# magenta/ddsp

Hardware: NVIDIA H100
Metric: audio samples/sec (Harmonic+FilteredNoise decoder) (higher is better)
Workload: dtype f32

## Files before the change

ddsp_b200/csrc/capi.cu:

```cuda
#include <stdarg.h>
#include <string.h>

#include <algorithm>

#include "common.cuh"
#include "controls.cuh"
#include "harmonic.cuh"
#include "harmonic_common.cuh"
#include "harmonic_v4.cuh"
#include "noise.cuh"
#include "noise_fused.cuh"
#include "noise_ring.cuh"
#include "host_pipeline.cuh"
#include "backward.cuh"
#include "harmonic_bwd2.cuh"
#include "controls_bwd.cuh"
#include "oscbank.cuh"
#include "sinusoidal.cuh"
#include "longconv.cuh"
#include "spectral.cuh"

namespace ddsp {

static thread_local char g_err[512] = "";
// ... 790 lines not shown
  const size_t z = (size_t)B * g.n_in * lc::M, h = (size_t)ir_batch * g.P * lc::M,
               w = (size_t)B * g.w_len;
  return sizeof(float2) * (z + h + w) + 256;
}

int ddsp_b200_fft_convolve_lti(const float* audio, const float* impulse_response,
                               float* out, int B, int N, int S, int ir_batch,
                               int start, int out_len, int accumulate, int flags,
                               void* workspace, size_t workspace_bytes, void* stream) {
  DDSP_REQUIRE(audio && impulse_response && out, DDSP_B200_E_INVALID,
               "fft_convolve_lti: null pointer");
  DDSP_REQUIRE(B >= 0 && N >= 1 && S >= 1, DDSP_B200_E_INVALID,
               "fft_convolve_lti: bad shape B=%d N=%d S=%d", B, N, S);
  DDSP_REQUIRE(ir_batch == B || ir_batch == 1, DDSP_B200_E_INVALID,
               "Batch size of audio (%d) and impulse response (%d) must be the same.",
               B, ir_batch);
  DDSP_REQUIRE(start >= 0 && out_len >= 0 &&
                   (long long)start + out_len <= (long long)N + S - 1,
               DDSP_B200_E_INVALID,
               "fft_convolve_lti: crop [%d, %d) leaves the convolution of length %lld",
               start, start + out_len, (long long)N + S - 1);
  if (B == 0 || out_len == 0) return 0;
  DDSP_REQUIRE(B <= 65535, DDSP_B200_E_INVALID,
               "fft_convolve_lti: B=%d exceeds the 65535 grid limit", B);
  const size_t need = ddsp_b200_fft_convolve_lti_workspace(B, N, S, ir_batch);
  DDSP_REQUIRE(workspace != nullptr && workspace_bytes >= need, DDSP_B200_E_WORKSPACE,
               "fft_convolve_lti: workspace of %zu B needed, %zu given", need,
               workspace_bytes);
  const lc::Geom g = lc::geom(N, S);
  float2* Z = reinterpret_cast<float2*>(((uintptr_t)workspace + 255) & ~(uintptr_t)255);
  float2* H = Z + (size_t)B * g.n_in * lc::M;
  float2* W = H + (size_t)ir_batch * g.P * lc::M;
  cudaStream_t st = (cudaStream_t)stream;
  DDSP_REQUIRE((flags & ~3) == 0, DDSP_B200_E_INVALID,
               "fft_convolve_lti: bad flags %d", flags);
  lc::lc_fft_blocks<<<dim3(g.P, ir_batch), lc::THREADS, 0, st>>>(
      impulse_response, H, S, 0, g.P, 1, (flags & DDSP_B200_LTI_REVERSE_IR) ? 1 : 0);
  DDSP_CHECK_LAUNCH("fft_convolve_lti(ir spectra)");
  lc::lc_fft_blocks<<<dim3(g.n_in, B), lc::THREADS, 0, st>>>(
      audio, Z, N, g.n2, g.n_in, 0, (flags & DDSP_B200_LTI_REVERSE_AUDIO) ? 1 : 0);
  DDSP_CHECK_LAUNCH("fft_convolve_lti(audio spectra)");
  const int lo_pos = std::max(0, start - g.n2);
  const int hi_pos = std::min(g.w_len, start + out_len);
  const int j_first = lo_pos / lc::L;
  const int j_last = std::min(g.n_out - 1, (hi_pos - 1) / lc::L);
  const int n_blocks = j_last - j_first + 1;
  {
    int rc = set_smem(lc::lc_mac_ifft, lc::kMacSmem, "fft_convolve_lti");
    if (rc) return rc;
  }
  lc::lc_mac_ifft<<<dim3((n_blocks + lc::JT - 1) / lc::JT, B), lc::THREADS, lc::kMacSmem,
                    st>>>(
      Z, H, W, g.n_in, g.P, g.n_out, ir_batch == 1 ? 0 : g.P * lc::M, j_first, n_blocks);
  DDSP_CHECK_LAUNCH("fft_convolve_lti(multiply-accumulate + inverse)");
  const int cgrid = std::min((out_len + 255) / 256, 8 * num_sms());
  lc::lc_combine<<<dim3(cgrid, B), 256, 0, st>>>(W, out, g.n2, g.w_len, start, out_len,
                                               N + S - 1, accumulate, j_first * lc::L,
                                               (j_last + 1) * lc::L);
  DDSP_CHECK_LAUNCH("fft_convolve_lti(combine)");
  return 0;
}

int ddsp_b200_angular_cumsum(const float* angular_frequency, float* phase, int B,
                             int N, int C, int chunk_size, int mode,
                             void* workspace, size_t workspace_bytes, void* stream) {
  DDSP_REQUIRE(angular_frequency && phase, DDSP_B200_E_INVALID,
               "angular_cumsum: null pointer");
  DDSP_REQUIRE(B >= 0 && N >= 1 && C >= 1, DDSP_B200_E_INVALID,
               "angular_cumsum: bad shape B=%d N=%d C=%d", B, N, C);
  DDSP_REQUIRE(mode >= 0 && mode <= 2, DDSP_B200_E_INVALID,
               "angular_cumsum: bad mode %d", mode);
  DDSP_REQUIRE(mode != 2 || chunk_size >= 1, DDSP_B200_E_INVALID,
               "angular_cumsum: chunk_size must be positive");
  if (B == 0) return 0;
  cudaStream_t st = (cudaStream_t)stream;
  if (mode != 0) {
    const int64_t BC = (int64_t)B * C;
    tf_sequential_cumsum<<<(int)((BC + 127) / 128), 128, 0, st>>>(
        angular_frequency, nullptr, phase, B, N, C, mode, chunk_size, 0, 1.0f);
    DDSP_CHECK_LAUNCH("angular_cumsum(tf_sequential)");
    return 0;
  }
  DDSP_REQUIRE(B <= 65535, DDSP_B200_E_INVALID,
               "angular_cumsum: B=%d exceeds the 65535 grid limit", B);
  const size_t need = ddsp_b200_oscillator_bank_workspace(B, N, C);
  DDSP_REQUIRE(workspace != nullptr && workspace_bytes >= need, DDSP_B200_E_WORKSPACE,
               "angular_cumsum: workspace of %zu B needed, %zu given", need,
               workspace_bytes);
  unsigned long long* sums = reinterpret_cast<unsigned long long*>(
      ((uintptr_t)workspace + 255) & ~(uintptr_t)255);
  const int n_chunks = (N + kObChunk - 1) / kObChunk;
  const double inv_two_pi = 0.15915494309189535;
  dim3 grid(n_chunks, B);
  oscbank_chunk_sums<<<grid, kObThreads, 0, st>>>(angular_frequency, sums, N, C,
                                                 n_chunks, inv_two_pi);
  DDSP_CHECK_LAUNCH("angular_cumsum(chunk sums)");
  const int64_t BK = (int64_t)B * C;
  oscbank_scan_chunks<<<(int)((BK + kObThreads - 1) / kObThreads), kObThreads, 0, st>>>(
      sums, C, n_chunks, BK);
  DDSP_CHECK_LAUNCH("angular_cumsum(scan)");
  oscbank_phase_out<<<grid, kObThreads, 0, st>>>(angular_frequency, sums, phase, N, C,
                                                n_chunks, inv_two_pi);
  DDSP_CHECK_LAUNCH("angular_cumsum(apply)");
  return 0;
}

int ddsp_b200_oscillator_bank_tf_sequential(const float* frequency_envelopes,
                                            const float* amplitude_envelopes,
                                            float* out, int B, int N, int K,
                                            float sample_rate, int use_angular_cumsum,
                                            int chunk_size, void* stream) {
  DDSP_REQUIRE(frequency_envelopes && amplitude_envelopes && out, DDSP_B200_E_INVALID,
               "oscillator_bank_tf_sequential: null pointer");
  DDSP_REQUIRE(B >= 0 && N >= 1 && K >= 1 && chunk_size >= 1 && sample_rate > 0.f,
               DDSP_B200_E_INVALID, "oscillator_bank_tf_sequential: bad arguments");
  if (B == 0) return 0;
  const int64_t BK = (int64_t)B * K;
  tf_sequential_cumsum<<<(int)((BK + 127) / 128), 128, 0, (cudaStream_t)stream>>>(
      frequency_envelopes, amplitude_envelopes, out, B, N, K,
      use_angular_cumsum ? 2 : 1, chunk_size, 1, sample_rate);
  DDSP_CHECK_LAUNCH("oscillator_bank_tf_sequential");
  return 0;
}

static int sinus_tile_frames(int F, int K) {
  int FT = std::min(16, F);
  while (FT > 1 && sf_smem(FT, K).total > kMaxDynSmem) FT = (FT + 1) / 2;
  return FT;
}

size_t ddsp_b200_sinusoidal_workspace(int B, int F, int K) {
  if (B <= 0 || F <= 0 || K <= 0) return 0;
  const int FT = sinus_tile_frames(F, K);
  const size_t n_tiles = ((size_t)F + FT - 1) / FT;
  return sizeof(unsigned long long) * (size_t)B * n_tiles * K + 256;
}

int ddsp_b200_sinusoidal_forward(const float* frequencies, const float* amplitudes,
                                 float* audio, int B, int F, int K, int N,
                                 float sample_rate, int amp_method, int accumulate,
                                 void* workspace, size_t workspace_bytes,
                                 void* stream) {
  DDSP_REQUIRE(frequencies && amplitudes && audio, DDSP_B200_E_INVALID,
               "sinusoidal_forward: null pointer");
  DDSP_REQUIRE(B >= 0 && F >= 1 && K >= 1 && N >= 1, DDSP_B200_E_INVALID,
               "sinusoidal_forward: bad shape B=%d F=%d K=%d N=%d", B, F, K, N);
  DDSP_REQUIRE(amp_method == DDSP_B200_AMP_WINDOW || amp_method == DDSP_B200_AMP_LINEAR,
               DDSP_B200_E_INVALID, "sinusoidal_forward: bad amp_method %d", amp_method);
  DDSP_REQUIRE(N % F == 0, DDSP_B200_E_INVALID,
               "sinusoidal_forward: n_samples (%d) must be divisible by the number "
               "of frames (%d)", N, F);
  DDSP_REQUIRE(amp_method != DDSP_B200_AMP_WINDOW || F < N, DDSP_B200_E_INVALID,
               "sinusoidal_forward: window upsampling cannot downsample (frames %d "
               ">= timesteps %d)", F, N);
  DDSP_REQUIRE(sample_rate > 0.f, DDSP_B200_E_INVALID,
               "sinusoidal_forward: sample_rate must be positive");
  if (B == 0) return 0;
  DDSP_REQUIRE(B <= 65535, DDSP_B200_E_INVALID,
               "sinusoidal_forward: B=%d exceeds the 65535 grid limit", B);
  const int FT = sinus_tile_frames(F, K);
  const SfSmem L = sf_smem(FT, K);
  DDSP_REQUIRE(L.total <= kMaxDynSmem, DDSP_B200_E_UNSUPPORTED,
               "sinusoidal_forward: K=%d needs more shared memory than one CTA has", K);
  const size_t need = ddsp_b200_sinusoidal_workspace(B, F, K);
  DDSP_REQUIRE(workspace != nullptr && workspace_bytes >= need, DDSP_B200_E_WORKSPACE,
               "sinusoidal_forward: workspace of %zu B needed, %zu given", need,
               workspace_bytes);
  unsigned long long* sums = reinterpret_cast<unsigned long long*>(
      ((uintptr_t)workspace + 255) & ~(uintptr_t)255);
  const int n_tiles = (F + FT - 1) / FT;
  const int hop = N / F;
  const double inv_sr = 1.0 / (double)sample_rate;
  cudaStream_t st = (cudaStream_t)stream;
  dim3 grid(n_tiles, B);
  sinus_tile_sums<<<grid, kSfThreads, 0, st>>>(frequencies, sums, F, K, hop, FT, n_tiles,
                                              inv_sr);
  DDSP_CHECK_LAUNCH("sinusoidal_forward(tile sums)");
  const int64_t BK = (int64_t)B * K;
  oscbank_scan_chunks<<<(int)((BK + kObThreads - 1) / kObThreads), kObThreads, 0, st>>>(
      sums, K, n_tiles, BK);
  DDSP_CHECK_LAUNCH("sinusoidal_forward(scan)");
  if (amp_method == DDSP_B200_AMP_WINDOW) {
    int rc = set_smem(sinus_apply<true>, L.total, "sinusoidal_forward");
    if (rc) return rc;
    sinus_apply<true><<<grid, kSfThreads, L.total, st>>>(
        frequencies, amplitudes, sums, audio, F, K, N, hop, FT, n_tiles, inv_sr,
        sample_rate * 0.5f, accumulate);
  } else {
    int rc = set_smem(sinus_apply<false>, L.total, "sinusoidal_forward");
    if (rc) return rc;
    sinus_apply<false><<<grid, kSfThreads, L.total, st>>>(
        frequencies, amplitudes, sums, audio, F, K, N, hop, FT, n_tiles, inv_sr,
        sample_rate * 0.5f, accumulate);
  }
  DDSP_CHECK_LAUNCH("sinusoidal_forward(apply)");
  return 0;
}

int ddsp_b200_resample(const float* in, float* out, int B, int F, int C, int N,
                       int method, int add_endpoint, void* stream) {
  DDSP_REQUIRE(in && out, DDSP_B200_E_INVALID, "resample: null pointer");
  DDSP_REQUIRE(B >= 0 && F >= 1 && C >= 1 && N >= 1, DDSP_B200_E_INVALID,
               "resample: bad shape B=%d F=%d C=%d N=%d", B, F, C, N);
  DDSP_REQUIRE(method >= 0 && method <= 3, DDSP_B200_E_INVALID,
               "resample: bad method %d", method);
  if (method == 0) {
    const int n_frames = add_endpoint ? F + 1 : F;
    const int n_intervals = n_frames - 1;
    DDSP_REQUIRE(n_frames < N, DDSP_B200_E_INVALID,
                 "Upsample with windows cannot be used for downsampling"
                 "More input frames (%d) than output timesteps (%d)", n_frames, N);
    DDSP_REQUIRE(n_intervals > 0 && N % n_intervals == 0, DDSP_B200_E_INVALID,
                 "For upsampling, the target the number of timesteps must be "
                 "divisible by the number of input frames%s. (timesteps:%d, "
                 "frames:%d, add_endpoint=%s).", add_endpoint ? "" : " - 1", N,
                 n_frames, add_endpoint ? "True" : "False");
  }
  if (B == 0) return 0;
  const int64_t total = (int64_t)B * N * C;
  resample_kernel<<<grid_for(total, 256, 16), 256, 0, (cudaStream_t)stream>>>(
      in, out, B, F, C, N, method, add_endpoint);
  DDSP_CHECK_LAUNCH("resample");
  return 0;
}

int ddsp_b200_add(const float* a, const float* b, float* out, int64_t n,
                  void* stream) {
  DDSP_REQUIRE(a && b && out, DDSP_B200_E_INVALID, "add: null pointer");
  DDSP_REQUIRE(n >= 0, DDSP_B200_E_INVALID, "add: n < 0");
  if (n == 0) return 0;
  add_kernel<<<grid_for(n, 256), 256, 0, (cudaStream_t)stream>>>(a, b, out, n);
  DDSP_CHECK_LAUNCH("add");
  return 0;
}


int ddsp_b200_frame_window(const float* audio, const float* window, float* frames,
                           int B, int N, int n_frames, int frame_size, int frame_step,
                           void* stream) {
  DDSP_REQUIRE(audio && window && frames, DDSP_B200_E_INVALID, "frame_window: null pointer");
  DDSP_REQUIRE(B >= 0 && N >= 1 && n_frames >= 1 && frame_size >= 4 && frame_size % 4 == 0 &&
                   frame_step >= 1 && B <= 65535,
               DDSP_B200_E_INVALID, "frame_window: bad shape B=%d N=%d T=%d n=%d step=%d", B,
               N, n_frames, frame_size, frame_step);
  DDSP_REQUIRE((((uintptr_t)window | (uintptr_t)frames) & 15) == 0, DDSP_B200_E_INVALID,
               "frame_window: window / frames must be 16-byte aligned");
  if (B == 0) return 0;
  const long long quads = ((long long)n_frames * frame_size) / 4;
  dim3 grid((unsigned)((quads + 255) / 256), B);
  frame_window_kernel<<<grid, 256, 0, (cudaStream_t)stream>>>(audio, window, frames, N, n_frames,
                                                            frame_size, frame_step);
  DDSP_CHECK_LAUNCH("frame_window");
  return 0;
}

int ddsp_b200_frame_window_adjoint(const float* grad_frames, const float* window,
                                   float* grad_audio, int B, int N, int n_frames,
                                   int frame_size, int frame_step,
                                   const float* scale_device, int accumulate,
                                   void* stream) {
  DDSP_REQUIRE(grad_frames && window && grad_audio, DDSP_B200_E_INVALID,
               "frame_window_adjoint: null pointer");
  DDSP_REQUIRE(B >= 0 && N >= 1 && n_frames >= 1 && frame_size >= 1 && frame_step >= 1 &&
                   B <= 65535,
               DDSP_B200_E_INVALID, "frame_window_adjoint: bad shape");
  if (B == 0) return 0;
  dim3 grid((N + 255) / 256, B);
  frame_window_adjoint_kernel<<<grid, 256, 0, (cudaStream_t)stream>>>(
      grad_frames, window, grad_audio, N, n_frames, frame_size, frame_step,
      scale_device, accumulate);
  DDSP_CHECK_LAUNCH("frame_window_adjoint");
  return 0;
}

int ddsp_b200_spectral_l1(const float* stft_target, const float* stft_value,
                          float* grad_value, double* sums, int64_t n_bins_total,
                          float mag_weight, float logmag_weight, int n_bins,
                          int irfft_size, void* stream) {
  DDSP_REQUIRE(stft_target && stft_value && grad_value && sums, DDSP_B200_E_INVALID,
               "spectral_l1: null pointer");
  DDSP_REQUIRE(n_bins_total >= 1 && n_bins >= 1 && n_bins_total % n_bins == 0 &&
                   (irfft_size == 0 || irfft_size == -1 || irfft_size == 2 * (n_bins - 1)),
               DDSP_B200_E_INVALID, "spectral_l1: bad sizes (total %lld, bins %d, irfft %d)",
               (long long)n_bins_total, n_bins, irfft_size);
  DDSP_REQUIRE((((uintptr_t)stft_target | (uintptr_t)stft_value | (uintptr_t)grad_value) & 15) == 0,
               DDSP_B200_E_INVALID, "spectral_l1: tensors must be 16-byte aligned");
  const long long blocks = std::min<long long>((n_bins_total / 2 + 255) / 256 + 1, 8ll * num_sms());
  spectral_l1_kernel<<<(unsigned)blocks, 256, 0, (cudaStream_t)stream>>>(
      reinterpret_cast<const float2*>(stft_target), reinterpret_cast<const float2*>(stft_value),
      reinterpret_cast<float2*>(grad_value), sums, n_bins_total, mag_weight, logmag_weight,
      1.0f / (float)n_bins_total, 1e-5f, n_bins, irfft_size);
  DDSP_CHECK_LAUNCH("spectral_l1");
  return 0;
}

#ifdef DDSP_NR_TIMING
int ddsp_b200_debug_noise_timing(unsigned* host_out) {
  cudaError_t e = cudaMemcpyFromSymbol(host_out, ddsp::nr_::g_nr_timing,
                                       sizeof(unsigned) * kMaxSMs * 32 * 8);
  return e == cudaSuccess ? 0 : DDSP_B200_E_CUDA;
}
#endif

}
```

ddsp_b200/csrc/harmonic_v4.cuh:

```cuda
#pragma once
#include "harmonic_common.cuh"

namespace ddsp {
namespace hv4 {

#ifndef DDSP_HV4_NW
#define DDSP_HV4_NW 1
#endif
constexpr int NW = DDSP_HV4_NW;
constexpr int NT = NW * 32;

#ifndef DDSP_HV4_PHASE_F64
#define DDSP_HV4_PHASE_F64 0
#endif
#ifndef DDSP_HV4_MIN_CTAS
#define DDSP_HV4_MIN_CTAS (24 / DDSP_HV4_NW)
#endif

constexpr double kMagic = 1572864.0 + 0.001953125;

struct __align__(16) FrameRec {
  unsigned long long P, A;
  unsigned long long D;
  int ng;
  int rem;
  float f_lo, f_hi, amp0, amp1;
};
static_assert(sizeof(FrameRec) == 48, "FrameRec must be three 16-byte words");

struct Smem {
  size_t off_mbar, off_sin, off_cos, off_x, off_w, off_red, off_inv, off_rec, off_live, total;
};

__host__ __device__ inline Smem smem_layout(int FW, int Kp, int hop) {
  Smem s;
  const size_t FT = (size_t)FW * NW;
  size_t o = 0;
  s.off_mbar = o; o += 16;
  s.off_sin = o;  o += sizeof(float) * kSinTab;
  s.off_cos = o;  o += sizeof(float) * kSinTab;
  s.off_x = o;    o += sizeof(float) * (FT + 1) * Kp;
  s.off_w = o;    o += (hop == 64) ? 0 : sizeof(float) * hop;
  o = (o + 15) & ~(size_t)15;
  s.off_red = o;  o += 16 * NW;
  s.off_rec = o;  o += sizeof(FrameRec) * FT;
  s.off_inv = o;  o += sizeof(float) * (FT + 1);
  s.off_live = o; o += sizeof(int) * (FT + 1);
  s.total = (o + 15) & ~(size_t)15;
  return s;
}

using hcm::phase32;

__device__ __forceinline__ float2 bffma2(float x, float2 v, float2 acc) {
  return ffma2(make_float2(x, x), v, acc);
}
__device__ __forceinline__ float2 bfmul2(float x, float2 v) {
  return fmul2(make_float2(x, x), v);
}

__device__ __forceinline__ void controls_rows4(float* __restrict__ sXw,
                                               const int* __restrict__ sLive,
                                               float* __restrict__ sInv, int r0,
                                               int nrows, int Kp, bool raw_scale,
                                               int lane) {
  const int K4 = Kp >> 2;
  const int sub = lane >> 3, l8 = lane & 7;
  const int r = r0 + sub;
  const bool row_ok = r < nrows;
  float4* row4 = reinterpret_cast<float4*>(sXw + (row_ok ? r : r0) * Kp);
  const int live = row_ok ? sLive[r] : 0;
  const int live4 = (live + 3) >> 2;
  float sum = 0.f;
  int c4 = l8;
  for (; c4 < live4; c4 += 8) {
    float4 x = row4[c4];
    if (raw_scale) {
      x.x = exp_sigmoid_f(x.x); x.y = exp_sigmoid_f(x.y);
      x.z = exp_sigmoid_f(x.z); x.w = exp_sigmoid_f(x.w);
    }
    const int k = 4 * c4;
    if (k + 1 >= live) x.y = 0.f;
    if (k + 2 >= live) x.z = 0.f;
    if (k + 3 >= live) x.w = 0.f;
    sum += (x.x + x.y) + (x.z + x.w);
    row4[c4] = x;
  }
  if (row_ok) {
    const float4 z = make_float4(0.f, 0.f, 0.f, 0.f);
    for (; c4 < K4; c4 += 8) row4[c4] = z;
  }
  sum += __shfl_xor_sync(0xffffffffu, sum, 4);
  sum += __shfl_xor_sync(0xffffffffu, sum, 2);
  sum += __shfl_xor_sync(0xffffffffu, sum, 1);
  if (row_ok && l8 == 0) sInv[r] = __fdividef(1.0f, (sum == 0.0f) ? 1e-7f : sum);
}

__device__ __noinline__ float sample_exact(const float* x0, int row_stride, float w0,
                                           float w1, uint32_t p32, float f_lo, float f_hi,
                                           float frac, int K, float nyq) {
  return harmonic_sample_exact(x0, x0 + row_stride, w0, w1, p32, f_lo, f_hi, frac, K, nyq);
}

struct Osc2 {
  float2 vo, ve, dlo, dle, na, sg;
  float2 s0e, s0o, s1e, s1o;
  float2 t0e, t0o, t1e, t1o;
};

__device__ __forceinline__ void osc_seed2(Osc2& st, uint32_t qa, uint32_t qb,
                                          const float* __restrict__ sSin,
                                          const float* __restrict__ sCos) {
  const uint32_t ia = qa >> (32 - kSinTabBits), ib = qb >> (32 - kSinTabBits);
  const float2 tx = make_float2(sSin[ia], sSin[ib]);
  const float2 ty = make_float2(sCos[ia], sCos[ib]);
  constexpr uint32_t kLow = (1u << (32 - kSinTabBits)) - 1u;
  constexpr float kC = 1.4629180792671596e-9f;
  constexpr float kOff = -(float)(1u << (31 - kSinTabBits)) * kC;
  const float2 eps = ffma2(make_float2((float)(qa & kLow), (float)(qb & kLow)),
                                make_float2(kC, kC), make_float2(kOff, kOff));
  const float2 e2 = fmul2(eps, eps);
  const float2 ce = ffma2(e2, make_float2(-0.5f, -0.5f), make_float2(1.f, 1.f));
  const float2 se = fmul2(eps, ffma2(e2, make_float2(-0.16666667f, -0.16666667f),
                                               make_float2(1.f, 1.f)));
  const float2 nse = make_float2(-se.x, -se.y);
  const float2 s1 = ffma2(ty, se, fmul2(tx, ce));
  const float2 c1 = ffma2(tx, nse, fmul2(ty, ce));
  const float2 ss = fmul2(s1, s1), cc = fmul2(c1, c1);
  const float2 s2 = fmul2(fadd2(s1, s1), c1);
  st.sg = make_float2(ss.x > cc.x ? -1.0f : 1.0f, ss.y > cc.y ? -1.0f : 1.0f);
  st.na = fmul2(make_float2(fminf(ss.x, cc.x), fminf(ss.y, cc.y)),
                     make_float2(-4.0f, -4.0f));
  st.vo = s1;
  st.ve = s2;
  st.dlo = ffma2(s1, st.sg, s1);
  st.dle = s2;
}

__device__ __forceinline__ void osc_step(Osc2& st) {
  st.dlo = ffma2(st.na, st.vo, st.dlo);
  st.dle = ffma2(st.na, st.ve, st.dle);
  st.vo = fadd2(st.vo, st.dlo);
  st.ve = fadd2(st.ve, st.dle);
}

__device__ __forceinline__ void osc_group(Osc2& st, const float4& X0, const float4& X1) {
  st.s0e = bffma2(X0.x, st.vo, st.s0e);
  st.s1e = bffma2(X1.x, st.vo, st.s1e);
  st.t0e = bffma2(X0.y, st.ve, st.t0e);
  st.t1e = bffma2(X1.y, st.ve, st.t1e);
  osc_step(st);
  st.s0o = bffma2(X0.z, st.vo, st.s0o);
  st.s1o = bffma2(X1.z, st.vo, st.s1o);
  st.t0o = bffma2(X0.w, st.ve, st.t0o);
  st.t1o = bffma2(X1.w, st.ve, st.t1o);
  osc_step(st);
}

__device__ __forceinline__ void osc_group_first(Osc2& st, const float4& X0,
                                                const float4& X1) {
  st.s0e = bfmul2(X0.x, st.vo);
  st.s1e = bfmul2(X1.x, st.vo);
  st.t0e = bfmul2(X0.y, st.ve);
  st.t1e = bfmul2(X1.y, st.ve);
  osc_step(st);
  st.s0o = bfmul2(X0.z, st.vo);
  st.s1o = bfmul2(X1.z, st.vo);
  st.t0o = bfmul2(X0.w, st.ve);
  st.t1o = bfmul2(X1.w, st.ve);
  osc_step(st);
}

__device__ __forceinline__ void osc_group_masked(Osc2& st, const float4& X0,
                                                 const float4& X1, int k, int ka,
                                                 int kb) {
  float2 mo = make_float2(k + 1 <= ka ? st.vo.x : 0.f, k + 1 <= kb ? st.vo.y : 0.f);
  float2 me = make_float2(k + 2 <= ka ? st.ve.x : 0.f, k + 2 <= kb ? st.ve.y : 0.f);
  st.s0e = bffma2(X0.x, mo, st.s0e);
  st.s1e = bffma2(X1.x, mo, st.s1e);
  st.t0e = bffma2(X0.y, me, st.t0e);
  st.t1e = bffma2(X1.y, me, st.t1e);
  osc_step(st);
  mo = make_float2(k + 3 <= ka ? st.vo.x : 0.f, k + 3 <= kb ? st.vo.y : 0.f);
  me = make_float2(k + 4 <= ka ? st.ve.x : 0.f, k + 4 <= kb ? st.ve.y : 0.f);
  st.s0o = bffma2(X0.z, mo, st.s0o);
  st.s1o = bffma2(X1.z, mo, st.s1o);
  st.t0o = bffma2(X0.w, me, st.t0o);
  st.t1o = bffma2(X1.w, me, st.t1o);
  osc_step(st);
}

__device__ __forceinline__ float4 mask4u(const float4& X, int rem) {
  return make_float4(X.x, rem > 1 ? X.y : 0.f, rem > 2 ? X.z : 0.f, 0.f);
}

struct LaneConst {
#if DDSP_HV4_PHASE_F64
  double c1a, c2a, c1b, c2b;
#else
  uint32_t c1a, c2a, c1b, c2b;
#endif
  float2 w1;
};

template <bool WINDOW>
__device__ __forceinline__ LaneConst lane_const(int r0, int lane, float inv_hop,
                                                const float* __restrict__ sW) {
  LaneConst c;
  const uint32_t ra = r0 + lane, rb = ra + 32;
#if DDSP_HV4_PHASE_F64
  c.c1a = (double)(ra + 1); c.c2a = (double)((ra * (ra + 1)) >> 1);
  c.c1b = (double)(rb + 1); c.c2b = (double)((rb * (rb + 1)) >> 1);
#else
  c.c1a = ra + 1; c.c2a = (ra * (ra + 1)) >> 1;
  c.c1b = rb + 1; c.c2b = (rb * (rb + 1)) >> 1;
#endif
#if DDSP_HV4_PHASE_F64
  asm volatile("" : "+d"(c.c1a), "+d"(c.c2a), "+d"(c.c1b), "+d"(c.c2b));
#else
  asm volatile("" : "+r"(c.c1a), "+r"(c.c2a), "+r"(c.c1b), "+r"(c.c2b));
#endif
  if (sW != nullptr) {
    c.w1 = make_float2(sW[ra], sW[rb]);
  } else {
    const float fa = (float)ra * inv_hop, fb = (float)rb * inv_hop;
    c.w1 = make_float2(WINDOW ? (0.5f - 0.5f * cospif(fa)) : fa,
                       WINDOW ? (0.5f - 0.5f * cospif(fb)) : fb);
  }
  asm volatile("" : "+f"(c.w1.x), "+f"(c.w1.y));
  return c;
}

__device__ __forceinline__ void frame_chunk(
    const float* __restrict__ sX, int xoff, int Kp, const FrameRec* __restrict__ rec,
    const LaneConst& lc, int r0, float inv_hop, const float* __restrict__ sSin,
    const float* __restrict__ sCos, int K, float nyquist, int lane,
    float* __restrict__ out, int accumulate) {
  const float* __restrict__ x0 = sX + xoff;
  const float* __restrict__ x1 = x0 + Kp;
  const ulonglong2 PA = *reinterpret_cast<const ulonglong2*>(&rec->P);
  const uint4 Dk = *reinterpret_cast<const uint4*>(&rec->D);
  const float4 fa = *reinterpret_cast<const float4*>(&rec->f_lo);
  const unsigned long long D = ((unsigned long long)Dk.y << 32) | Dk.x;
  const int ng = (int)Dk.z, rem = (int)Dk.w;
#if DDSP_HV4_PHASE_F64
  const double Pd = __longlong_as_double((long long)PA.x);
  const double Ad = __longlong_as_double((long long)PA.y);
  const double Dd = __longlong_as_double((long long)D);
  const uint32_t qa = (uint32_t)__double2loint(fma(lc.c2a, Dd, fma(lc.c1a, Ad, Pd)));
  const uint32_t qb = (uint32_t)__double2loint(fma(lc.c2b, Dd, fma(lc.c1b, Ad, Pd)));
#else
  const uint32_t qa = phase32(PA.x, PA.y, D, lc.c1a, lc.c2a);
  const uint32_t qb = phase32(PA.x, PA.y, D, lc.c1b, lc.c2b);
#endif
  const float2 w0 = ffma2(make_float2(-lc.w1.x, -lc.w1.y), make_float2(fa.z, fa.z),
                               make_float2(fa.z, fa.z));
  const float2 w1 = bfmul2(fa.w, lc.w1);
  float2 y;
  if (ng < 0) {
    constexpr uint32_t kRound = 1u << (31 - kSinTabBits);
    int ra = r0 + lane, xo = xoff;
    asm volatile("" : "+r"(ra), "+r"(xo));
    const float fra = (float)ra * inv_hop, frb = (float)(ra + 32) * inv_hop;
    y.x = sample_exact(sX + xo, Kp, w0.x, w1.x, qa - kRound, fa.x, fa.y, fra, K, nyquist);
    y.y = sample_exact(sX + xo, Kp, w0.y, w1.y, qb - kRound, fa.x, fa.y, frb, K, nyquist);
  } else {
    Osc2 st;
    osc_seed2(st, qa, qb, sSin, sCos);
    if (ng > 0) {
      st.s0e = st.s0o = st.s1e = st.s1o = make_float2(0.f, 0.f);
      st.t0e = st.t0o = st.t1e = st.t1o = make_float2(0.f, 0.f);
      const int k_main = ng << 2;
      int k = 0;
#pragma unroll 1
      do {
        const float4 X0 = *reinterpret_cast<const float4*>(x0 + k);
        const float4 X1 = *reinterpret_cast<const float4*>(x1 + k);
        osc_group(st, X0, X1);
        k += 4;
      } while (k < k_main);
      if (rem != 0) {
        const float4 X0 = mask4u(*reinterpret_cast<const float4*>(x0 + k), rem);
        const float4 X1 = mask4u(*reinterpret_cast<const float4*>(x1 + k), rem);
        osc_group(st, X0, X1);
      }
    } else {
      int ra = r0 + lane;
      asm volatile("" : "+r"(ra));
      const float fra = (float)ra * inv_hop, frb = (float)(ra + 32) * inv_hop;
      const int ka = live_harmonics(fa.x, fa.y, fra, K, nyquist);
      const int kb = live_harmonics(fa.x, fa.y, frb, K, nyquist);
      const int kmin = __reduce_min_sync(0xffffffffu, min(ka, kb));
      const int kmax = __reduce_max_sync(0xffffffffu, max(ka, kb));
      st.s0e = st.s0o = st.s1e = st.s1o = make_float2(0.f, 0.f);
      st.t0e = st.t0o = st.t1e = st.t1o = make_float2(0.f, 0.f);
      const int k_main = kmin & ~3;
      int k = 0;
      for (; k < k_main; k += 4) {
        const float4 X0 = *reinterpret_cast<const float4*>(x0 + k);
        const float4 X1 = *reinterpret_cast<const float4*>(x1 + k);
        osc_group(st, X0, X1);
      }
      for (; k < kmax; k += 4) {
        const float4 X0 = *reinterpret_cast<const float4*>(x0 + k);
        const float4 X1 = *reinterpret_cast<const float4*>(x1 + k);
        osc_group_masked(st, X0, X1, k, ka, kb);
      }
    }
    const float2 t0 = ffma2(st.sg, fadd2(st.s0o, st.t0o), fadd2(st.s0e, st.t0e));
    const float2 t1 = ffma2(st.sg, fadd2(st.s1o, st.t1o), fadd2(st.s1e, st.t1e));
    y = ffma2(t1, w1, fmul2(t0, w0));
  }
  if (accumulate) {
    y.x += out[0];
    y.y += out[32];
  }
  out[0] = y.x;
  out[32] = y.y;
}

template <bool WINDOW, int HOPT>
__global__ void __launch_bounds__(NT, DDSP_HV4_MIN_CTAS)
harmonic_v4_kernel(HarmonicParams p, int use_tma, int FW) {
  extern __shared__ __align__(16) unsigned char smem_raw[];
  const int hop = HOPT ? HOPT : p.hop;
  const int Kp = p.Kp, K = p.K, F = p.F;
  const int FT = FW * NW;
  const Smem L = smem_layout(FW, Kp, hop);
  void* mbar = (void*)(smem_raw + L.off_mbar);
  float* sSin = (float*)(smem_raw + L.off_sin);
  float* sCos = (float*)(smem_raw + L.off_cos);
  float* sX = (float*)(smem_raw + L.off_x);
  float* sW = (HOPT == 64) ? nullptr : (float*)(smem_raw + L.off_w);
  double* sRedD = (double*)(smem_raw + L.off_red);
  unsigned long long* sWarpTot = (unsigned long long*)(smem_raw + L.off_red) + NW;
  float* sInv = (float*)(smem_raw + L.off_inv);
  FrameRec* sRec = (FrameRec*)(smem_raw + L.off_rec);
  int* sLive = (int*)(smem_raw + L.off_live);

  const int b = blockIdx.y;
  const int i0 = blockIdx.x * FT;
  const int nfr = min(FT, F - i0);
  const int rows_in = min(nfr + 1, F - i0);
  const int tid = threadIdx.x, lane = tid & 31, warp = tid >> 5;
  const float* f0b = p.f0 + (size_t)b * F;
  const float* ampb = p.amps + (size_t)b * F;

  asm volatile("griddepcontrol.launch_dependents;" ::: "memory");
  if (use_tma && tid == 0) {
    mbar_init(mbar, 1);
    const uint32_t bytes = (uint32_t)rows_in * (uint32_t)K * 4u;
    mbar_expect_tx(mbar, bytes);
    tma_bulk_g2s(sX, p.hd + ((size_t)b * F + i0) * K, bytes, mbar);
  }

  const int n_rec = (FT + 31) >> 5;
  const bool rec_warp = warp < n_rec;
  const int fr = warp * 32 + lane;
  const int cnt = max(0, min(32, nfr - warp * 32));
  const bool raw_scale = p.ctl_flags & DDSP_B200_CTL_SCALE;
  float f = 0.f, a = 0.f, f_tile = 0.f, f_first = 0.f;
  float f_x = 0.f, a_x = 0.f;
  if (rec_warp && cnt > 0) {
    if (lane <= cnt) {
      const int g = min(i0 + fr, F - 1);
      f = f0b[g];
      a = ampb[g];
    }
    if (lane == 31 && cnt == 32) {
      const int g = min(i0 + fr + 1, F - 1);
      f_x = f0b[g];
      a_x = ampb[g];
    }
    f_tile = f0b[i0];
    f_first = f0b[0];
  }
  constexpr int TPT = kSinTab / NT;
  static_assert(TPT * NT == kSinTab, "the table splits evenly over the CTA");
  float2 tab[TPT];
#pragma unroll
  for (int u = 0; u < TPT; ++u) tab[u] = hcm::g_sincos256[tid + u * NT];
  double part = 0.0;
  if ((reinterpret_cast<uintptr_t>(f0b) & 15) == 0) {
    const float4* f4 = reinterpret_cast<const float4*>(f0b);
    const int n4 = i0 >> 2;
    float4 v[4];
    int j = tid;
    for (; j + 3 * NT < n4; j += 4 * NT) {
#pragma unroll
      for (int u = 0; u < 4; ++u) v[u] = f4[j + u * NT];
#pragma unroll
      for (int u = 0; u < 4; ++u)
        part += ((double)v[u].x + (double)v[u].y) + ((double)v[u].z + (double)v[u].w);
    }
#pragma unroll
    for (int u = 0; u < 4; ++u)
      v[u] = (j + u * NT < n4) ? f4[j + u * NT] : make_float4(0.f, 0.f, 0.f, 0.f);
    const float tail = (tid < (i0 & 3)) ? f0b[4 * n4 + tid] : 0.f;
#pragma unroll
    for (int u = 0; u < 4; ++u)
      part += ((double)v[u].x + (double)v[u].y) + ((double)v[u].z + (double)v[u].w);
    part += (double)tail;
  } else {
#pragma unroll 4
    for (int j = tid; j < i0; j += NT) part += (double)f0b[j];
  }
#pragma unroll
  for (int o = 16; o > 0; o >>= 1) part += __shfl_xor_sync(0xffffffffu, part, o);
  if (lane == 0) sRedD[warp] = part;
#pragma unroll
  for (int u = 0; u < TPT; ++u) {
    sSin[tid + u * NT] = tab[u].x;
    sCos[tid + u * NT] = tab[u].y;
  }
  const float inv_hop = 1.0f / (float)hop;
  if (HOPT != 64) {
    for (int r = tid; r < hop; r += NT) {
      const float frac = (float)r * inv_hop;
      sW[r] = WINDOW ? (0.5f - 0.5f * cospif(frac)) : frac;
    }
  }
  if (!use_tma) {
    if (p.hd != nullptr) {
      const float* hdb = p.hd + ((size_t)b * F + i0) * K;
      for (int idx = tid; idx < rows_in * Kp; idx += NT) {
        int r = idx / Kp, c = idx - r * Kp;
        sX[idx] = (c < K) ? hdb[r * K + c] : 0.f;
      }
    } else {
      for (int idx = tid; idx < rows_in * Kp; idx += NT)
        sX[idx] = (idx % Kp == 0) ? 1.0f : 0.f;
    }
  }

  const bool have_ctl = (p.ctl_flags != 0) && (p.hd != nullptr);
  const bool zero_ok = have_ctl && (p.ctl_flags & DDSP_B200_CTL_NYQUIST);
  unsigned long long excl = 0;
  if (rec_warp && cnt > 0) {
    if (raw_scale && lane <= cnt) a = exp_sigmoid_f(a);
    const float f_next = __shfl_down_sync(0xffffffffu, f, 1);
    const float a_next = __shfl_down_sync(0xffffffffu, a, 1);
    float f_n = f_next, a_n = a_next;
    if (lane == 31 && cnt == 32) {
      f_n = f_x;
      a_n = raw_scale ? exp_sigmoid_f(a_x) : a_x;
    }
    unsigned long long tot = 0;
    double a0 = 0.0, dd = 0.0;
    if (lane < cnt) {
      a0 = (double)f * p.inv_sr;
      const double a1 = (double)f_n * p.inv_sr;
      dd = (a1 - a0) * (1.0 / (double)hop);
      tot = turns_to_fix64((double)hop * a0 + (a1 - a0) * (0.5 * (hop - 1)));
    }
    unsigned long long incl = tot;
#pragma unroll
    for (int o = 1; o < 32; o <<= 1) {
      const unsigned long long up = __shfl_up_sync(0xffffffffu, incl, o);
      if (lane >= o) incl += up;
    }
    excl = incl - tot;
    if (lane == 31) sWarpTot[warp] = incl;
    auto row_live = [&](float fq) {
      int live = K;
      if ((p.ctl_flags & DDSP_B200_CTL_NYQUIST) && fq > 0.f) {
        int k = (int)fminf(p.nyquist / fq, (float)K);
        while (k < K && __fmul_rn(fq, (float)(k + 1)) < p.nyquist) ++k;
        while (k > 0 && !(__fmul_rn(fq, (float)k) < p.nyquist)) --k;
        live = k;
      }
      return live;
    };
    const int live = row_live(f);
    int live_next = __shfl_down_sync(0xffffffffu, live, 1);
    if (lane == 31 && cnt == 32) live_next = row_live(f_n);
    int ng = -1, rem = 0;
    if (lane < cnt && f >= 1.0f && f_n >= 1.0f) {
      const int kca = live_harmonics(f, f_n, 0.0f, K, p.nyquist);
      const int kcb = live_harmonics(f, f_n, (float)(hop - 1) * inv_hop, K, p.nyquist);
      ng = 0;
      if (kca == kcb) {
        if (zero_ok && live == kca && live_next <= kca) {
          ng = max(1, (kca + 3) >> 2);
        } else {
          ng = kca >> 2;
          rem = kca & 3;
        }
      }
    }
    if (lane < cnt) {
      FrameRec r;
#if DDSP_HV4_PHASE_F64
      r.P = 0;
      r.A = (unsigned long long)__double_as_longlong(a0);
      r.D = (unsigned long long)__double_as_longlong(dd);
#else
      r.P = 0; r.A = turns_to_fix64(a0); r.D = turns_to_fix64(dd);
#endif
      r.ng = ng; r.rem = rem;
      r.f_lo = f; r.f_hi = f_n; r.amp0 = a; r.amp1 = a_n;
      sRec[fr] = r;
    }
    if (lane <= cnt) sLive[fr] = live;
    if (lane == 31 && cnt == 32) sLive[fr + 1] = live_next;
  }
  __syncthreads();

  if (rec_warp && cnt > 0) {
    double base_sum = 0.0;
#pragma unroll
    for (int w = 0; w < NW; ++w) base_sum += sRedD[w];
    const double a_tile = (double)f_tile * p.inv_sr;
    const double a_first = (double)f_first * p.inv_sr;
    unsigned long long P0 = turns_to_fix64(
        (double)hop * (base_sum * p.inv_sr) + 0.5 * (hop - 1) * (a_tile - a_first));
    for (int w = 0; w < warp; ++w) P0 += sWarpTot[w];
    if (lane < cnt) {
      const unsigned long long Pf = P0 + excl;
#if DDSP_HV4_PHASE_F64
      const double Pd = (double)(Pf >> 11) * 1.1102230246251565e-16 + kMagic;
      sRec[fr].P = (unsigned long long)__double_as_longlong(Pd);
#else
      sRec[fr].P = Pf + 0x80000000ull + (1ull << (63 - kSinTabBits));
#endif
    }
  }
  if (use_tma) mbar_wait(mbar, 0);

  const int w0f = warp * FW;
  const int nfw = max(0, min(FW, nfr - w0f));
  if (nfw > 0) {
    float* sXw = sX + (size_t)w0f * Kp;
    const bool last = (w0f + nfw == nfr);
    int nrows = nfw;
    if (last && rows_in > nfr) nrows = nfw + 1;
    if (have_ctl) {
      if (Kp <= 128) {
        for (int r0 = 0; r0 < nrows; r0 += 4)
          controls_rows4(sXw, sLive + w0f, sInv + w0f, r0, nrows, Kp, raw_scale, lane);
      } else {
        for (int r0 = 0; r0 < nrows; r0 += 4)
          hcm::controls_rows(sXw, sLive + w0f, r0, nrows, Kp, raw_scale, lane);
        for (int r = lane; r < nrows; r += 32) sInv[w0f + r] = 1.0f;
      }
    } else {
      for (int r = lane; r < nrows; r += 32) sInv[w0f + r] = 1.0f;
    }
    if (last && rows_in < nfr + 1) {
      __syncwarp();
      for (int c = lane; c < Kp; c += 32) sXw[nfw * Kp + c] = sXw[(nfw - 1) * Kp + c];
      if (lane == 0) sInv[w0f + nfw] = sInv[w0f + nfw - 1];
    }
  }
  __syncthreads();

  if (nfw > 0) {
    FrameRec* rec = sRec + w0f;
    if (lane < nfw) {
      rec[lane].amp0 *= sInv[w0f + lane];
      rec[lane].amp1 *= sInv[w0f + lane + 1];
    }
    __syncwarp();
    float* o = p.audio + (size_t)b * p.N + (size_t)(i0 + w0f) * hop + lane;
    int xoff = w0f * Kp;
    if (HOPT == 64) {
      const LaneConst lc = lane_const<WINDOW>(0, lane, inv_hop, nullptr);
#pragma unroll 1
      for (int li = 0; li < nfw; ++li, ++rec, xoff += Kp, o += 64) {
        frame_chunk(sX, xoff, Kp, rec, lc, 0, inv_hop, sSin, sCos, K, p.nyquist, lane, o,
                    p.accumulate);
      }
    } else {
      for (int li = 0; li < nfw; ++li, ++rec, xoff += Kp) {
        for (int r0 = 0; r0 < hop; r0 += 64, o += 64) {
          const LaneConst lc = lane_const<WINDOW>(r0, lane, inv_hop, sW);
          frame_chunk(sX, xoff, Kp, rec, lc, r0, inv_hop, sSin, sCos, K, p.nyquist, lane, o,
                      p.accumulate);
        }
      }
    }
  }
}

template <bool WINDOW, int HOPT>
inline cudaError_t launch_one(const HarmonicParams& p, int use_tma, int FW, dim3 grid,
                              size_t smem, cudaStream_t st) {
  if (smem > 48 * 1024) {
    cudaError_t e = cudaFuncSetAttribute(harmonic_v4_kernel<WINDOW, HOPT>,
                                         cudaFuncAttributeMaxDynamicSharedMemorySize,
                                         (int)smem);
    if (e != cudaSuccess) return e;
  }
  harmonic_v4_kernel<WINDOW, HOPT><<<grid, NT, smem, st>>>(p, use_tma, FW);
  return cudaSuccess;
}

}

inline int launch_harmonic_v4(HarmonicParams p, cudaStream_t st) {
  using namespace hv4;
  p.Kp = (p.K + 3) & ~3;
  static const int env_fw = [] { const char* e = getenv("DDSP_B200_HARM_FW"); return e ? atoi(e) : 0; }();
  int FW = (NW == 1) ? 11 : 8;
  const long long want_ctas = 8ll * num_sms() * (4 / NW);
  while (FW > 4 && (long long)p.B * ((p.F + FW * NW - 1) / (FW * NW)) < want_ctas) FW = (FW + 1) >> 1;
  while (FW > 1 && (long long)p.B * ((p.F + FW * NW - 1) / (FW * NW)) < num_sms()) FW = (FW + 1) >> 1;
  if (env_fw > 0) FW = std::min(32, env_fw);
  FW = std::max(1, std::min(FW, (p.F + NW - 1) / NW));
  while (FW > 1 && smem_layout(FW, p.Kp, p.hop).total > 64 * 1024) FW = (FW + 1) / 2;
  const size_t smem = smem_layout(FW, p.Kp, p.hop).total;
  if (smem > 200 * 1024) return 1;
  const int use_tma = (p.hd != nullptr) && (p.K % 4 == 0) &&
                      (((uintptr_t)p.hd & 15) == 0);
  dim3 grid((p.F + FW * NW - 1) / (FW * NW), p.B);
  cudaError_t e;
  const bool win = p.amp_method == DDSP_B200_AMP_WINDOW;
  if (p.hop == 64) {
    e = win ? launch_one<true, 64>(p, use_tma, FW, grid, smem, st)
            : launch_one<false, 64>(p, use_tma, FW, grid, smem, st);
  } else {
    e = win ? launch_one<true, 0>(p, use_tma, FW, grid, smem, st)
            : launch_one<false, 0>(p, use_tma, FW, grid, smem, st);
  }
  if (e != cudaSuccess) {
    (void)cudaGetLastError();
    set_error("harmonic_forward(v4): %s", cudaGetErrorString(e));
    return DDSP_B200_E_CUDA;
  }
  DDSP_CHECK_LAUNCH("harmonic_forward(v4)");
  return 0;
}

}
```

Before: 43.72 billion.

## Split record and controls work across warps, use 4-warp CTAs, unroll oscillator loads

Raises the default harmonic CTA to four warps. Frame-record building now runs on a subset of warps that sync through a named barrier, while the remaining warps compute per-row live-harmonic counts and normalise the controls in parallel, overlapping that work with the TMA wait. The inner oscillator loop now uses raw shared-memory vector loads, peels the first group and unrolls by two to cut loop overhead and address arithmetic. It also adds optional clock-based per-phase timing instrumentation. The added barriers and extra warps change occupancy and may add synchronisation cost.

Result: faster. 46.49 billion, median of 6 (+6.3%).

```diff
diff --git a/ddsp_b200/csrc/capi.cu b/ddsp_b200/csrc/capi.cu
--- a/ddsp_b200/csrc/capi.cu
+++ b/ddsp_b200/csrc/capi.cu
@@ -1116,4 +1116,17 @@
 }
 #endif
 
-}
+#ifdef DDSP_HV4_TIMING
+int ddsp_b200_debug_harm_timing(unsigned long long* host_out) {
+  const size_t bytes = sizeof(unsigned long long) * kMaxSMs * (ddsp::hv4::kTimingPhases + 1);
+  cudaError_t e = cudaMemcpyFromSymbol(host_out, ddsp::hv4::g_hv4_timing, bytes);
+  if (e != cudaSuccess) return DDSP_B200_E_CUDA;
+  void* dev = nullptr;
+  e = cudaGetSymbolAddress(&dev, ddsp::hv4::g_hv4_timing);
+  if (e == cudaSuccess) e = cudaMemset(dev, 0, bytes);
+  if (e == cudaSuccess) e = cudaDeviceSynchronize();
+  return e == cudaSuccess ? 0 : DDSP_B200_E_CUDA;
+}
+#endif
+
+}
diff --git a/ddsp_b200/csrc/harmonic_v4.cuh b/ddsp_b200/csrc/harmonic_v4.cuh
--- a/ddsp_b200/csrc/harmonic_v4.cuh
+++ b/ddsp_b200/csrc/harmonic_v4.cuh
@@ -5,7 +5,7 @@
 namespace hv4 {
 
 #ifndef DDSP_HV4_NW
-#define DDSP_HV4_NW 1
+#define DDSP_HV4_NW 4
 #endif
 constexpr int NW = DDSP_HV4_NW;
 constexpr int NT = NW * 32;
@@ -15,6 +15,34 @@
 #endif
 #ifndef DDSP_HV4_MIN_CTAS
 #define DDSP_HV4_MIN_CTAS (24 / DDSP_HV4_NW)
+#endif
+
+#ifdef DDSP_HV4_TIMING
+constexpr int kTimingPhases = 8;
+__device__ unsigned long long g_hv4_timing[kMaxSMs * (kTimingPhases + 1)];
+#define HV4_TIMING_DECL                                                                 \
+  unsigned tacc__[kTimingPhases] = {0, 0, 0, 0, 0, 0, 0, 0};                            \
+  unsigned tprev__ = (unsigned)clock()
+#define HV4_LAP(i)                                                                      \
+  do {                                                                                  \
+    const unsigned n__ = (unsigned)clock();                                             \
+    tacc__[i] += n__ - tprev__;                                                         \
+    tprev__ = n__;                                                                      \
+  } while (0)
+#define HV4_TIMING_FLUSH()                                                              \
+  do {                                                                                  \
+    if (lane == 0) {                                                                    \
+      unsigned smid__;                                                                  \
+      asm volatile("mov.u32 %0, %%smid;" : "=r"(smid__));                               \
+      unsigned long long* t__ = g_hv4_timing + (smid__ % kMaxSMs) * (kTimingPhases + 1); \
+      for (int i__ = 0; i__ < kTimingPhases; ++i__) atomicAdd(t__ + i__, (unsigned long long)tacc__[i__]); \
+      atomicAdd(t__ + kTimingPhases, 1ull);                                             \
+    }                                                                                   \
+  } while (0)
+#else
+#define HV4_TIMING_DECL
+#define HV4_LAP(i)
+#define HV4_TIMING_FLUSH()
 #endif
 
 constexpr double kMagic = 1572864.0 + 0.001953125;
@@ -51,6 +79,14 @@
 }
 
 using hcm::phase32;
+
+__device__ __forceinline__ float4 lds128(uint32_t a) {
+  float4 v;
+  asm volatile("ld.shared.v4.f32 {%0, %1, %2, %3}, [%4];"
+               : "=f"(v.x), "=f"(v.y), "=f"(v.z), "=f"(v.w)
+               : "r"(a));
+  return v;
+}
 
 __device__ __forceinline__ float2 bffma2(float x, float2 v, float2 acc) {
   return ffma2(make_float2(x, x), v, acc);
@@ -94,6 +130,17 @@
   sum += __shfl_xor_sync(0xffffffffu, sum, 2);
   sum += __shfl_xor_sync(0xffffffffu, sum, 1);
   if (row_ok && l8 == 0) sInv[r] = __fdividef(1.0f, (sum == 0.0f) ? 1e-7f : sum);
+}
+
+__device__ __forceinline__ int row_live_count(float fq, int K, float nyquist, bool nyq) {
+  int live = K;
+  if (nyq && fq > 0.f) {
+    int k = (int)fminf(nyquist / fq, (float)K);
+    while (k < K && __fmul_rn(fq, (float)(k + 1)) < nyquist) ++k;
+    while (k > 0 && !(__fmul_rn(fq, (float)k) < nyquist)) --k;
+    live = k;
+  }
+  return live;
 }
 
 __device__ __noinline__ float sample_exact(const float* x0, int row_stride, float w0,
@@ -237,7 +284,7 @@
     const float* __restrict__ sCos, int K, float nyquist, int lane,
     float* __restrict__ out, int accumulate) {
   const float* __restrict__ x0 = sX + xoff;
-  const float* __restrict__ x1 = x0 + Kp;
+  const uint32_t kp4 = (uint32_t)Kp << 2;
   const ulonglong2 PA = *reinterpret_cast<const ulonglong2*>(&rec->P);
   const uint4 Dk = *reinterpret_cast<const uint4*>(&rec->D);
   const float4 fa = *reinterpret_cast<const float4*>(&rec->f_lo);
@@ -268,22 +315,21 @@
     Osc2 st;
     osc_seed2(st, qa, qb, sSin, sCos);
     if (ng > 0) {
-      st.s0e = st.s0o = st.s1e = st.s1o = make_float2(0.f, 0.f);
-      st.t0e = st.t0o = st.t1e = st.t1o = make_float2(0.f, 0.f);
-      const int k_main = ng << 2;
-      int k = 0;
+      uint32_t a = smem_u32(x0);
+      const uint32_t a_end = a + (ng << 4);
+      osc_group_first(st, lds128(a), lds128(a + kp4));
+      a += 16;
+      if ((ng & 1) == 0) {
+        osc_group(st, lds128(a), lds128(a + kp4));
+        a += 16;
+      }
 #pragma unroll 1
-      do {
-        const float4 X0 = *reinterpret_cast<const float4*>(x0 + k);
-        const float4 X1 = *reinterpret_cast<const float4*>(x1 + k);
-        osc_group(st, X0, X1);
-        k += 4;
-      } while (k < k_main);
-      if (rem != 0) {
-        const float4 X0 = mask4u(*reinterpret_cast<const float4*>(x0 + k), rem);
-        const float4 X1 = mask4u(*reinterpret_cast<const float4*>(x1 + k), rem);
-        osc_group(st, X0, X1);
-      }
+      while (a != a_end) {
+        osc_group(st, lds128(a), lds128(a + kp4));
+        osc_group(st, lds128(a + 16), lds128(a + kp4 + 16));
+        a += 32;
+      }
+      if (rem != 0) osc_group(st, mask4u(lds128(a), rem), mask4u(lds128(a + kp4), rem));
     } else {
       int ra = r0 + lane;
       asm volatile("" : "+r"(ra));
@@ -294,18 +340,20 @@
       const int kmax = __reduce_max_sync(0xffffffffu, max(ka, kb));
       st.s0e = st.s0o = st.s1e = st.s1o = make_float2(0.f, 0.f);
       st.t0e = st.t0o = st.t1e = st.t1o = make_float2(0.f, 0.f);
-      const int k_main = kmin & ~3;
-      int k = 0;
-      for (; k < k_main; k += 4) {
-        const float4 X0 = *reinterpret_cast<const float4*>(x0 + k);
-        const float4 X1 = *reinterpret_cast<const float4*>(x1 + k);
-        osc_group(st, X0, X1);
-      }
-      for (; k < kmax; k += 4) {
-        const float4 X0 = *reinterpret_cast<const float4*>(x0 + k);
-        const float4 X1 = *reinterpret_cast<const float4*>(x1 + k);
-        osc_group_masked(st, X0, X1, k, ka, kb);
-      }
+      uint32_t a = smem_u32(x0);
+      const uint32_t a_main = a + ((kmin & ~3) << 2);
+      if (kmin & 4) {
+        osc_group(st, lds128(a), lds128(a + kp4));
+        a += 16;
+      }
+#pragma unroll 1
+      while (a != a_main) {
+        osc_group(st, lds128(a), lds128(a + kp4));
+        osc_group(st, lds128(a + 16), lds128(a + kp4 + 16));
+        a += 32;
+      }
+      for (int k = kmin & ~3; k < kmax; k += 4, a += 16)
+        osc_group_masked(st, lds128(a), lds128(a + kp4), k, ka, kb);
     }
     const float2 t0 = ffma2(st.sg, fadd2(st.s0o, st.t0o), fadd2(st.s0e, st.t0e));
     const float2 t1 = ffma2(st.sg, fadd2(st.s1o, st.t1o), fadd2(st.s1e, st.t1e));
@@ -347,6 +395,7 @@
   const float* ampb = p.amps + (size_t)b * F;
 
   asm volatile("griddepcontrol.launch_dependents;" ::: "memory");
+  HV4_TIMING_DECL;
   if (use_tma && tid == 0) {
     mbar_init(mbar, 1);
     const uint32_t bytes = (uint32_t)rows_in * (uint32_t)K * 4u;
@@ -359,6 +408,14 @@
   const int fr = warp * 32 + lane;
   const int cnt = max(0, min(32, nfr - warp * 32));
   const bool raw_scale = p.ctl_flags & DDSP_B200_CTL_SCALE;
+  const int n_ctl = (NW > n_rec) ? NW - n_rec : NW;
+  const int cw = (NW > n_rec) ? warp - n_rec : warp;
+  const int rw = (nfr + n_ctl - 1) / n_ctl;
+  const int c0 = cw * rw;
+  const int ncr = (cw < 0) ? 0 : max(0, min(rw, nfr - c0));
+  const bool c_last = ncr > 0 && c0 + ncr == nfr;
+  const int nrows = ncr + ((c_last && rows_in > nfr) ? 1 : 0);
+  const float f_row = (lane < nrows) ? f0b[min(i0 + c0 + lane, F - 1)] : 0.f;
   float f = 0.f, a = 0.f, f_tile = 0.f, f_first = 0.f;
   float f_x = 0.f, a_x = 0.f;
   if (rec_warp && cnt > 0) {
@@ -432,6 +489,9 @@
         sX[idx] = (idx % Kp == 0) ? 1.0f : 0.f;
     }
   }
+  HV4_LAP(0);
+  __syncthreads();
+  HV4_LAP(1);
 
   const bool have_ctl = (p.ctl_flags != 0) && (p.hd != nullptr);
   const bool zero_ok = have_ctl && (p.ctl_flags & DDSP_B200_CTL_NYQUIST);
@@ -461,19 +521,10 @@
     }
     excl = incl - tot;
     if (lane == 31) sWarpTot[warp] = incl;
-    auto row_live = [&](float fq) {
-      int live = K;
-      if ((p.ctl_flags & DDSP_B200_CTL_NYQUIST) && fq > 0.f) {
-        int k = (int)fminf(p.nyquist / fq, (float)K);
-        while (k < K && __fmul_rn(fq, (float)(k + 1)) < p.nyquist) ++k;
-        while (k > 0 && !(__fmul_rn(fq, (float)k) < p.nyquist)) --k;
-        live = k;
-      }
-      return live;
-    };
-    const int live = row_live(f);
+    const bool nyq = p.ctl_flags & DDSP_B200_CTL_NYQUIST;
+    const int live = row_live_count(f, K, p.nyquist, nyq);
     int live_next = __shfl_down_sync(0xffffffffu, live, 1);
-    if (lane == 31 && cnt == 32) live_next = row_live(f_n);
+    if (lane == 31 && cnt == 32) live_next = row_live_count(f_n, K, p.nyquist, nyq);
     int ng = -1, rem = 0;
     if (lane < cnt && f >= 1.0f && f_n >= 1.0f) {
       const int kca = live_harmonics(f, f_n, 0.0f, K, p.nyquist);
@@ -501,12 +552,10 @@
       r.f_lo = f; r.f_hi = f_n; r.amp0 = a; r.amp1 = a_n;
       sRec[fr] = r;
     }
-    if (lane <= cnt) sLive[fr] = live;
-    if (lane == 31 && cnt == 32) sLive[fr + 1] = live_next;
-  }
-  __syncthreads();
-
-  if (rec_warp && cnt > 0) {
+    const int n_act = (nfr + 31) >> 5;
+    if (n_act > 1) asm volatile("bar.sync 1, %0;" ::"r"(32 * n_act) : "memory");
+    HV4_LAP(2);
+
     double base_sum = 0.0;
 #pragma unroll
     for (int w = 0; w < NW; ++w) base_sum += sRedD[w];
@@ -525,35 +574,43 @@
 #endif
     }
   }
-  if (use_tma) mbar_wait(mbar, 0);
-
-  const int w0f = warp * FW;
-  const int nfw = max(0, min(FW, nfr - w0f));
-  if (nfw > 0) {
-    float* sXw = sX + (size_t)w0f * Kp;
-    const bool last = (w0f + nfw == nfr);
-    int nrows = nfw;
-    if (last && rows_in > nfr) nrows = nfw + 1;
+  HV4_LAP(3);
+
+  if (ncr > 0) {
+    float* sXw = sX + (size_t)c0 * Kp;
+    if (have_ctl) {
+      const bool nyq = p.ctl_flags & DDSP_B200_CTL_NYQUIST;
+      for (int r = lane; r < nrows; r += 32)
+        sLive[c0 + r] = row_live_count(r == lane ? f_row : f0b[min(i0 + c0 + r, F - 1)], K,
+                                       p.nyquist, nyq);
+      __syncwarp();
+    }
+    if (use_tma) mbar_wait(mbar, 0);
+    HV4_LAP(4);
     if (have_ctl) {
       if (Kp <= 128) {
         for (int r0 = 0; r0 < nrows; r0 += 4)
-          controls_rows4(sXw, sLive + w0f, sInv + w0f, r0, nrows, Kp, raw_scale, lane);
+          controls_rows4(sXw, sLive + c0, sInv + c0, r0, nrows, Kp, raw_scale, lane);
       } else {
         for (int r0 = 0; r0 < nrows; r0 += 4)
-          hcm::controls_rows(sXw, sLive + w0f, r0, nrows, Kp, raw_scale, lane);
-        for (int r = lane; r < nrows; r += 32) sInv[w0f + r] = 1.0f;
+          hcm::controls_rows(sXw, sLive + c0, r0, nrows, Kp, raw_scale, lane);
+        for (int r = lane; r < nrows; r += 32) sInv[c0 + r] = 1.0f;
       }
     } else {
-      for (int r = lane; r < nrows; r += 32) sInv[w0f + r] = 1.0f;
-    }
-    if (last && rows_in < nfr + 1) {
+      for (int r = lane; r < nrows; r += 32) sInv[c0 + r] = 1.0f;
+    }
+    if (c_last && rows_in < nfr + 1) {
       __syncwarp();
-      for (int c = lane; c < Kp; c += 32) sXw[nfw * Kp + c] = sXw[(nfw - 1) * Kp + c];
-      if (lane == 0) sInv[w0f + nfw] = sInv[w0f + nfw - 1];
-    }
-  }
+      for (int c = lane; c < Kp; c += 32) sXw[ncr * Kp + c] = sXw[(ncr - 1) * Kp + c];
+      if (lane == 0) sInv[c0 + ncr] = sInv[c0 + ncr - 1];
+    }
+  }
+  HV4_LAP(5);
   __syncthreads();
-
+  HV4_LAP(6);
+
+  const int w0f = warp * FW;
+  const int nfw = max(0, min(FW, nfr - w0f));
   if (nfw > 0) {
     FrameRec* rec = sRec + w0f;
     if (lane < nfw) {
@@ -580,6 +637,8 @@
       }
     }
   }
+  HV4_LAP(7);
+  HV4_TIMING_FLUSH();
 }
 
 template <bool WINDOW, int HOPT>
```
